# rezashkv/unlearn-ft

Hardware: AMD Instinct MI355X
Metric: bilevel train-step images/sec @512^2 pruned-SD2.1 (higher is better)
Workload: dtype bf16; 1 GPU; BASELINE configs[1] model+batch (MAC-budget-0.55 SD-2.1 student [ratio 0.556, 223.7 GMAC/img] + dense teacher [402.1 GMAC/img], B=8/GPU, 64x64 latents = 512^2 px, losses 1.0 ddpm(min-SNR 5) + 2.0 distill + 0.1 block) under the bilevel cadence of configs[2] (upper concept-suppression step every 10th iteration, second AdamW); global_batch=8, parallelism=dp1, student_params=483766084, weights=random-init, attention_precision=activation dtype, dist_backend=none, rccl_ranks=0, dp_mode=allreduce, teacher_prefetch=True

## Files before the change

include/pdmk.h:

```cpp
#ifndef PDMK_H
#define PDMK_H
#include <stdint.h>
#ifdef __cplusplus
extern "C" {
#endif

#define PDMK_F32 0
#define PDMK_BF16 1

typedef void* pdmk_stream;

int pdmk_version(void);

#define PDMK_A_ROWK 0
#define PDMK_A_CONV 1
#define PDMK_A_COLK 2
#define PDMK_B_ROWK 0
#define PDMK_B_COLK 1
#define PDMK_B_COLK_CONV 2

typedef struct pdmk_gemm_args {
    const void* A;
    const void* B;
    void* C;
// ... 24 lines not shown
    void* ln_out;
    int32_t ld_ln_out;
    float ln_eps;
} pdmk_gemm_args;
int pdmk_gemm_ln_supported(const pdmk_gemm_args* args);

#define PDMK_EPI_NONE 0
#define PDMK_EPI_GEGLU 1
#define PDMK_EPI_GEGLU_BWD 2

int pdmk_gemm(const pdmk_gemm_args* args, pdmk_stream stream);
int pdmk_conv_up2_supported(int B, int H, int W, int Ci, int Co, int dtype);
int pdmk_groupnorm_apply_colstat(const void* x, void* y, const float* gamma, const float* beta, float* stats, const int64_t* colstat,
                                 int cs_ld, int cs_col0, int B, int HW, int C, int ldx, int ldy, int G, int gs, float eps,
                                 int silu, int dtype, pdmk_stream stream);
int pdmk_up2_pack_weights(const float* w3, void* wp, void* wpt, int Co, int Ci, int dtype, pdmk_stream stream);
int pdmk_up2_combine_wgrad(const float* dwp, float* dw3, int Co, int Ci, pdmk_stream stream);
#define PDMK_COLSTAT_SCALE 1073741824.0
#define PDMK_GEMM_GROUP_MAX 8
int pdmk_gemm_group(const pdmk_gemm_args* args, int n, pdmk_stream stream, int32_t* grouped_out);
int pdmk_gemm_plan(const pdmk_gemm_args* args, pdmk_stream stream, int32_t* splitk_out);
int pdmk_gemm_last_candidate(void);
int pdmk_gemm_candidate_name(int a_mode, int b_mode, int id, char* buf, int n);
int pdmk_splitk_finish(const float* ws, void* C, const float* bias, const float* rowvec, const void* R, int64_t M,
                       int N, int ldc, int ldr, int rows_per_b, int ldrv , int nslab ,
                       int accumulate, int dtype, pdmk_stream stream);
int pdmk_splitk_finish_colstat(const float* ws, void* C, const float* bias, const float* rowvec, const void* R, int64_t M,
                               int N, int ldc, int ldr, int rows_per_b, int ldrv, int nslab, int accumulate, int64_t* colstat,
                               int cs_ld, int cs_col0, int dtype, pdmk_stream stream);
#define PDMK_SLAB_GROUP_MAX 32
typedef struct pdmk_slab_item {
    const float* ws;
    float* dst;
    int64_t n;
    int32_t nslab, pad_;
} pdmk_slab_item;
int pdmk_splitk_finish_group(const pdmk_slab_item* items, int n_items, pdmk_stream stream);
int64_t pdmk_gemm_splitk_workspace_bytes(int64_t M, int N, int splitk);

int pdmk_plan_export(const char* path);
int pdmk_plan_import(const char* path);
int pdmk_plan_size(void);
int pdmk_plan_clear(void);
int pdmk_debug_scratch_violations(void);

int pdmk_groupnorm_fwd(const void* x, void* y, const float* gamma, const float* beta, float* stats, double* ws,
// ... 159 lines not shown
```

unlearn-ft_amd/csrc/gemm.hip:

```cpp
#include <cstdio>
#include <cstdlib>
#include <cstring>
#include <map>
#include <mutex>
#include <vector>

#include "common.h"
#include <algorithm>

namespace {

#define PDMK_GEMM_NBUF 2
#ifndef PDMK_GEMM_PF2
#define PDMK_GEMM_PF2 0
#endif
constexpr int BM = 128, BN = 128;
template <typename T, int KCHUNKS, int NW> struct TileCfg {
    static constexpr int NTHREADS = 64 * NW;
    static constexpr int IM = 8 / NW * 2;
    static constexpr int TPR = NTHREADS / 128;
    static constexpr int NLD = KCHUNKS / TPR;
    static constexpr int ROW_BYTES = KCHUNKS == 8 ? 144 : 96;
    static constexpr int OPERAND_BYTES = 128 * ROW_BYTES;
    static constexpr int CH = Mma<T>::CH;
// ... 406 lines not shown
        }
    } else if (g.a_mode == PDMK_A_COLK && g.b_mode == PDMK_B_COLK) PDMK_GO(PDMK_A_COLK, PDMK_B_COLK, 0);
    else if (g.a_mode == PDMK_A_COLK && g.b_mode == PDMK_B_COLK_CONV) {
        switch (g.conv_mode) {
            case 0: PDMK_GO(PDMK_A_COLK, PDMK_B_COLK_CONV, 0); break;
            case 1: PDMK_GO(PDMK_A_COLK, PDMK_B_COLK_CONV, 1); break;
            case 2: PDMK_GO(PDMK_A_COLK, PDMK_B_COLK_CONV, 2); break;
            default: return -2;
        }
    } else return -2;
#undef PDMK_GO
    PDMK_CHECK_LAUNCH();
    return 0;
}

}

int pdmk_gemm_dma_launch(const pdmk_gemm_args& g, hipStream_t st, long a_bytes, long b_bytes);
int pdmk_gemm_ring_launch(const pdmk_gemm_args& g, hipStream_t st, long a_bytes, long b_bytes, int id);
int pdmk_gemm_ring_num_configs();
int pdmk_gemm_ring_pick(const pdmk_gemm_args& g);
int pdmk_wgrad_ring_launch(const pdmk_gemm_args& g, hipStream_t st, long a_bytes, long b_bytes, int id);
int pdmk_wgrad_ring_num_configs();

static int env_int(const char* name, int def, int* cache) {
    static int dynamic = -1;
    if (dynamic < 0) dynamic = getenv("PDMK_ENV_DYNAMIC") ? 1 : 0;
    if (*cache == INT32_MIN || dynamic) {
        const char* e = getenv(name);
        *cache = e ? atoi(e) : def;
    }
    return *cache;
}
static int dma_mode() { static int c = INT32_MIN; return env_int("PDMK_GEMM_DMA", 1, &c); }
static int ring_mode() { static int c = INT32_MIN; return env_int("PDMK_GEMM_RING", 1, &c); }
static int tune_mode() { static int c = INT32_MIN; return env_int("PDMK_GEMM_TUNE", 1, &c); }
static int forced_cfg() { static int c = INT32_MIN; return env_int("PDMK_RING_CFG", -1, &c); }
static int forced_wcfg() { static int c = INT32_MIN; return env_int("PDMK_WGRAD_CFG", -1, &c); }

namespace {

struct PlanKey {
    int v[10];
    bool operator<(const PlanKey& o) const { return memcmp(v, o.v, sizeof v) < 0; }
};
std::mutex g_plan_mu;
// ... 443 lines not shown
        char* base = reinterpret_cast<char*>(g_scratch) + off[i];
        t[i].C = base;
        t[i].ldc = a[i].N;
        t[i].colstat = nullptr;
        if (t[i].epilogue == PDMK_EPI_GEGLU_BWD) t[i].ldc = 2 * a[i].N;
        else t[i].C2 = nullptr;
        if (t[i].accumulate == 1) t[i].accumulate = 0;
        if (t[i].epilogue == PDMK_EPI_GEGLU) t[i].ldc = a[i].N / 2;
        if (t[i].colsum_out)
            t[i].colsum_out = reinterpret_cast<float*>(base + (off[i + 1] - off[i]) - (((size_t)a[i].M * 4 + 15) & ~(size_t)15));
    }
    hipEvent_t e0, e1;
    if (hipEventCreate(&e0) != hipSuccess || hipEventCreate(&e1) != hipSuccess) { (void)hipGetLastError(); return -1; }
    const float t_sep = time_us([&]() -> int {
        for (int i = 0; i < n; ++i) {
            int rc = launch_candidate(t[i], st, ids[i]);
            if (rc == 1) rc = launch_legacy(t[i], st);
            if (rc) return rc;
        }
        return 0;
    }, st, e0, e1);
    int best = -1;
    float bt = t_sep * 0.98f;
    int cands[PDMK_GEMM_GROUP_MAX + 12], nc = 0;
    for (int i = 0; i < n; ++i) cands[nc++] = ids[i];
    cands[nc++] = heuristic_cfg(a[0]);
    if (a[0].a_mode == PDMK_A_CONV)
        for (int h = 0; h < 4; ++h) cands[nc++] = 1 + 12 + h;
    if (a[0].a_mode == PDMK_A_COLK && a[0].b_mode == PDMK_B_COLK)
        for (int w = 0; w < 5; ++w) cands[nc++] = 1 + w;
    for (int i = 0; i < nc; ++i) {
        bool seen = cands[i] <= 0;
        for (int j = 0; j < i; ++j) seen = seen || cands[j] == cands[i];
        if (seen) continue;
        const float tg = time_us([&]() -> int { return group_launch(t, n, st, cands[i]); }, st, e0, e1);
        if (tg < bt) { bt = tg; best = cands[i]; }
    }
    (void)hipEventDestroy(e0);
    (void)hipEventDestroy(e1);
    if (getenv("PDMK_TUNE_LOG")) {
        fprintf(stderr, "[pdmk group] n=%d", n);
        for (int i = 0; i < n; ++i) fprintf(stderr, " (%d,%d,%d|a%d sk%d id%d)", a[i].M, a[i].N, a[i].K, a[i].a_mode, a[i].splitk, ids[i]);
        fprintf(stderr, " separate %.1f us -> %s %d (%.1f us)\n", t_sep, best > 0 ? "grouped cand" : "separate", best, best > 0 ? bt : t_sep);
    }
    {
        std::lock_guard<std::mutex> lk(g_plan_mu);
        if (!scratch_check()) return -1;
    }
    return best;
}

}

// ... 46 lines not shown
        if (can_tune(st)) {
            id = tune_group(a, n, ids, st);
            std::lock_guard<std::mutex> lk(g_plan_mu);
            g_group_plan[key] = id;
        } else {
            id = ids[0];
            for (int i = 1; i < n; ++i)
                if (ids[i] != ids[0]) id = -1;
        }
    }
    if (id > 0) {
        const int rc = group_launch(a, n, st, id);
        if (rc == 0) {
            g_last_candidate = id;
            if (grouped_out) *grouped_out = n;
            return 0;
        }
        if (rc != 1) return rc;
    }
    return separate();
}

extern "C" int pdmk_gemm_last_candidate(void) { return g_last_candidate; }
int pdmk_gemm_ring_name(int id, int conv, char* buf, int n);
int pdmk_wgrad_ring_name(int id, int conv, char* buf, int n);
extern "C" int pdmk_gemm_candidate_name(int a_mode, int b_mode, int id, char* buf, int n) {
    if (!buf || n <= 0) return -1;
    if (id <= 0) {
        snprintf(buf, n, "igemm_kernel / pdmk_dma::igemm_dma_kernel (K-step-32)");
        return 0;
    }
    if (a_mode == PDMK_A_COLK) return pdmk_wgrad_ring_name(id - 1, b_mode == PDMK_B_COLK_CONV, buf, n);
    return pdmk_gemm_ring_name(id - 1, a_mode == PDMK_A_CONV, buf, n);
}

extern "C" int pdmk_gemm_plan(const pdmk_gemm_args* a, pdmk_stream stream, int32_t* splitk_out) {
    if (!a || !splitk_out) return -1;
    const pdmk_gemm_args& g = *a;
    hipStream_t st = reinterpret_cast<hipStream_t>(stream);
    *splitk_out = 1;
    if (g.M <= 0 || g.N <= 0 || g.K <= 0) return -1;
    if ((g.N & 3) || g.epilogue) return 0;
    const bool wg = wgrad_eligible(g);
    if (g.a_mode == PDMK_A_COLK && !wg) {
        *splitk_out = heuristic_wgrad_sk(g);
        return 0;
// ... 69 lines not shown
        if (kind == 'c') g_plan_cfg[k] = val;
        else if (kind == 's') g_plan_sk[k] = val;
        ++n;
    }
    fclose(f);
    return n;
}
extern "C" int pdmk_plan_clear(void) {
    std::lock_guard<std::mutex> lk(g_plan_mu);
    g_plan_cfg.clear();
    g_plan_sk.clear();
    g_group_plan.clear();
    if (g_scratch) (void)hipFree(g_scratch);
    g_scratch = nullptr;
    g_scratch_bytes = 0;
    return 0;
}

extern "C" int pdmk_debug_scratch_violations(void) {
    std::lock_guard<std::mutex> lk(g_plan_mu);
    return g_scratch_violations;
}

extern "C" int pdmk_version(void) { return 121; }
```

unlearn-ft_amd/csrc/gemm_ring.hip:

```cpp
#include "common.h"

#include <stdio.h>
#include <stdlib.h>

#ifndef PDMK_WGRAD_XCD
#define PDMK_WGRAD_XCD 1
#endif
#ifndef PDMK_HALO_PAIRS
#define PDMK_HALO_PAIRS 1
#endif
#ifndef PDMK_RING_SPLIT_ISSUE
#define PDMK_RING_SPLIT_ISSUE 0
#endif
#ifndef PDMK_HALO_SPLIT_ISSUE
#define PDMK_HALO_SPLIT_ISSUE 1
#endif

#ifndef PDMK_PRIO
#define PDMK_PRIO 0
#endif

namespace pdmk_ring {

constexpr int BK = 64, NT = 512;
constexpr unsigned OOB = 0x80000000u;
typedef __attribute__((address_space(3))) void lds_void;
// ... 916 lines not shown
        for (int i = 0; i < IM; ++i) {
            const int m = m0 + wm * (16 * IM) + i * 16 + (lane & 15);
            if (m < g.M) unsafeAtomicAdd(g.colsum_out + m, acs[i][0]);
        }
    }
    ring_epilogue<BM, NJ, STAGES * SLOT>(g, wgc, acc, smem, m0, n0);
}

template <bool CONV, int BM, int NJ, int STAGES, int OCC>
__global__ __launch_bounds__(NT, OCC) void wgrad_ring_kernel(pdmk_gemm_args g, int lg_wo, int lg_howo, unsigned a_bytes,
                                                             unsigned b_bytes) {
    __shared__ __attribute__((aligned(1024))) unsigned char smem[wgrad_smem_bytes(BM, NJ, STAGES)];
    wgrad_ring_body<CONV, BM, NJ, STAGES, OCC>(g, lg_wo, lg_howo, a_bytes, b_bytes, PDMK_WGRAD_XCD ? lc_split_xcd() : lc_plain(), smem);
}
template <bool CONV, int BM, int NJ, int STAGES, int OCC>
__global__ __launch_bounds__(NT, OCC) void wgrad_ring_group_kernel(pdmk_gemm_group_dev gg) {
    __shared__ __attribute__((aligned(1024))) unsigned char smem[wgrad_smem_bytes(BM, NJ, STAGES)];
    int pi;
    LC wgc;
    if (!lc_group(gg, pi, wgc)) return;
    wgrad_ring_body<CONV, BM, NJ, STAGES, OCC>(gg.p[pi], gg.aux0[pi], gg.aux1[pi], gg.a_bytes[pi], gg.b_bytes[pi], wgc, smem);
}

struct Config {
    int bm, nj, stages, occ;
};
static const Config kConfigs[] = {
    {256, 4, 3, 2}, {256, 5, 3, 2}, {128, 4, 4, 2}, {128, 5, 4, 2}, {64, 4, 6, 2}, {64, 5, 5, 2},
    {128, 4, 2, 4}, {64, 4, 3, 4},  {64, 5, 2, 4},  {128, 6, 3, 2}, {64, 6, 4, 2},  {128, 5, 2, 4},
    {64, 2, 4, 4},  {128, 2, 3, 4}, {64, 3, 4, 4},
};
constexpr int kNumConfigs = sizeof(kConfigs) / sizeof(kConfigs[0]);
constexpr int kNumBase = 12;

static int halo_tile_w(const pdmk_gemm_args& g, int h, int splitk) {
    const bool phase = g.conv_mode >= 5 && g.conv_mode <= 13;
    if (g.a_mode != PDMK_A_CONV || !(g.conv_mode == 0 || phase) || g.conv_ho != g.conv_hi || g.conv_wo != g.conv_wi) return 0;
    if (phase && (h < 2 || !PDMK_HALO_PAIRS || g.R || (splitk > 1))) return 0;
    if ((g.conv_ci % 8) || g.conv_wi < 4) return 0;
    if (phase ? ((g.ldb % 8) || g.ldb < (g.conv_mode == 13 ? 16 : 4) * g.conv_ci) : g.ldb != 9 * g.conv_ci) return 0;
    if ((splitk > 1 ? splitk : 1) > (g.conv_ci + 63) / 64) return 0;
    const int bm = h < 2 ? 256 : 128, pmax = h < 2 ? 400 : 264;
    const int H = g.conv_hi, W = g.conv_wi, HW = H * W;
    if (HW < bm) return (bm % HW) == 0 && (bm / HW) * (H + 2) * (W + 2) <= pmax ? W : 0;
    if (HW % bm) return 0;
    static const int pref = getenv("PDMK_HALO_TW") ? atoi(getenv("PDMK_HALO_TW")) : 0;
// ... 417 lines not shown
        }
        return hipGetLastError() == hipSuccess ? 0 : -1000;
    }
    const Config c = kConfigs[id < kNumBase ? id : id - kNumHalo];
#define PDMK_RING_GGO(BMv, NJv, STv, OCv)                                                                             \
    case (BMv * 1000 + NJv * 100 + STv * 10 + OCv):                                                                   \
        if (conv) hipLaunchKernelGGL((igemm_ring_group_kernel<true, BMv, NJv, STv, OCv>), grid, dim3(NT), 0, st, G.gg); \
        else hipLaunchKernelGGL((igemm_ring_group_kernel<false, BMv, NJv, STv, OCv>), grid, dim3(NT), 0, st, G.gg);   \
        break;
    switch (c.bm * 1000 + c.nj * 100 + c.stages * 10 + c.occ) {
        PDMK_RING_GGO(256, 4, 3, 2) PDMK_RING_GGO(256, 5, 3, 2) PDMK_RING_GGO(128, 4, 4, 2) PDMK_RING_GGO(128, 5, 4, 2)
        PDMK_RING_GGO(64, 4, 6, 2) PDMK_RING_GGO(64, 5, 5, 2) PDMK_RING_GGO(128, 4, 2, 4) PDMK_RING_GGO(64, 4, 3, 4)
        PDMK_RING_GGO(64, 5, 2, 4) PDMK_RING_GGO(128, 6, 3, 2) PDMK_RING_GGO(64, 6, 4, 2) PDMK_RING_GGO(128, 5, 2, 4)
        PDMK_RING_GGO(64, 2, 4, 4) PDMK_RING_GGO(128, 2, 3, 4) PDMK_RING_GGO(64, 3, 4, 4)
        default: return 1;
    }
#undef PDMK_RING_GGO
    return hipGetLastError() == hipSuccess ? 0 : -1000;
}

struct WCfg { int bm, nj, stages, occ; };
static const WCfg kWCfgs[] = {{128, 4, 4, 2}, {128, 4, 2, 4}, {64, 4, 3, 4}, {128, 2, 3, 4}, {64, 2, 4, 4}};
constexpr int kNumW = sizeof(kWCfgs) / sizeof(kWCfgs[0]);
int pdmk_wgrad_ring_num_configs() { return kNumW + 2; }
int pdmk_wgrad_ring_name(int id, int conv, char* buf, int n) {
    if (id == kNumW || id == kNumW + 1) {
        snprintf(buf, n, "pdmk_ring::conv_wgrad_halo_kernel<%d, %d>", id == kNumW ? 2 : 4, id == kNumW ? 3 : 2);
        return 0;
    }
    if (id < 0 || id >= kNumW) return -1;
    const WCfg c = kWCfgs[id];
    snprintf(buf, n, "pdmk_ring::wgrad_ring_kernel<%s, %d, %d, %d, %d>", conv ? "true" : "false", c.bm, c.nj, c.stages, c.occ);
    return 0;
}
int pdmk_wgrad_ring_launch(const pdmk_gemm_args& g, hipStream_t st, long a_bytes, long b_bytes, int id) {
    using namespace pdmk_ring;
    if (g.dtype != PDMK_BF16 || g.a_mode != PDMK_A_COLK || g.b_mode == PDMK_B_ROWK || !g.out_f32) return 1;
    const bool conv = g.b_mode == PDMK_B_COLK_CONV;
    if ((g.M % 8) || (g.N % 8) || (g.lda % 8) || (!conv && (g.ldb % 8))) return 1;
    if (conv && ((g.conv_ci % 8) || (g.conv_ld % 8) || g.conv_mode == 3 || g.conv_mode == 4 || g.conv_mode > 8)) return 1;
    if (id == kNumW || id == kNumW + 1) {
        if (!wgrad_halo_ok(g)) return 1;
        const int nblk = (g.K + 127) / 128, sk = g.splitk > 1 ? g.splitk : 1, bm = id == kNumW ? 64 : 128;
        if (sk > nblk) return 1;
        dim3 grid(((g.M + bm - 1) / bm) * ((g.conv_ci + 63) / 64), sk);
        if (bm == 64) hipLaunchKernelGGL((conv_wgrad_halo_kernel<2, 3>), grid, dim3(NT), 0, st, g, (unsigned)a_bytes, (unsigned)b_bytes);
        else hipLaunchKernelGGL((conv_wgrad_halo_kernel<4, 2>), grid, dim3(NT), 0, st, g, (unsigned)a_bytes, (unsigned)b_bytes);
        return hipGetLastError() == hipSuccess ? 0 : -1000;
    }
    if (id < 0 || id >= kNumW) return 1;
    int lg_wo = -1, lg_howo = -1;
    if (conv) {
        auto lg = [](int v) { int l = 0; if (v <= 0 || (v & (v - 1))) return -1; while ((1 << l) < v) ++l; return l; };
        lg_wo = lg(g.conv_wo);
        lg_howo = lg(g.conv_ho * g.conv_wo);
        if (lg_wo < 0 || lg_howo < 0) lg_wo = lg_howo = -1;
    }
    const WCfg c = kWCfgs[id];
    const int bn = 32 * c.nj;
    dim3 grid(((g.M + c.bm - 1) / c.bm) * ((g.N + bn - 1) / bn), g.splitk > 1 ? g.splitk : 1);
#define PDMK_WG_GO(BMv, NJv, STv, OCv)                                                                                \
    case (BMv * 1000 + NJv * 100 + STv * 10 + OCv):                                                                   \
        if (conv) hipLaunchKernelGGL((wgrad_ring_kernel<true, BMv, NJv, STv, OCv>), grid, dim3(NT), 0, st, g, lg_wo,  \
                                     lg_howo, (unsigned)a_bytes, (unsigned)b_bytes);                                  \
        else hipLaunchKernelGGL((wgrad_ring_kernel<false, BMv, NJv, STv, OCv>), grid, dim3(NT), 0, st, g, lg_wo,      \
                                lg_howo, (unsigned)a_bytes, (unsigned)b_bytes);                                       \
        break;
    switch (c.bm * 1000 + c.nj * 100 + c.stages * 10 + c.occ) {
        PDMK_WG_GO(128, 4, 4, 2) PDMK_WG_GO(128, 4, 2, 4) PDMK_WG_GO(64, 4, 3, 4) PDMK_WG_GO(128, 2, 3, 4) PDMK_WG_GO(64, 2, 4, 4)
        default: return 1;
    }
#undef PDMK_WG_GO
    return hipGetLastError() == hipSuccess ? 0 : -1000;
}

int pdmk_wgrad_ring_group_launch(const pdmk_gemm_args* gs, int n, hipStream_t st, const long* a_bytes, const long* b_bytes, int id) {
    using namespace pdmk_ring;
    if (n < 2 || n > PDMK_GEMM_GROUP_MAX || id < 0 || id > kNumW + 1) return 1;
    const bool conv = gs[0].b_mode == PDMK_B_COLK_CONV;
    const bool halo = id == kNumW || id == kNumW + 1;
    GroupGrid G;
    for (int i = 0; i < n; ++i) {
        const pdmk_gemm_args& g = gs[i];
        if (g.dtype != PDMK_BF16 || g.a_mode != PDMK_A_COLK || g.b_mode == PDMK_B_ROWK || !g.out_f32) return 1;
        if ((g.b_mode == PDMK_B_COLK_CONV) != conv) return 1;
        if ((g.M % 8) || (g.N % 8) || (g.lda % 8) || (!conv && (g.ldb % 8))) return 1;
        if (conv && ((g.conv_ci % 8) || (g.conv_ld % 8) || g.conv_mode == 3 || g.conv_mode == 4 || g.conv_mode > 8)) return 1;
        const int sk = g.splitk > 1 ? g.splitk : 1;
        if (halo) {
            if (!wgrad_halo_ok(g)) return 1;
            const int nblk = (g.K + 127) / 128, bm = id == kNumW ? 64 : 128;
            if (sk > nblk) return 1;
            G.add(i, g, ((g.M + bm - 1) / bm) * ((g.conv_ci + 63) / 64), sk, a_bytes[i], b_bytes[i]);
        } else {
            int lg_wo = -1, lg_howo = -1;
            if (conv) {
                auto lg = [](int v) { int l = 0; if (v <= 0 || (v & (v - 1))) return -1; while ((1 << l) < v) ++l; return l; };
                lg_wo = lg(g.conv_wo);
                lg_howo = lg(g.conv_ho * g.conv_wo);
                if (lg_wo < 0 || lg_howo < 0) lg_wo = lg_howo = -1;
            }
            const WCfg c = kWCfgs[id];
            const int bn = 32 * c.nj;
            G.add(i, g, ((g.M + c.bm - 1) / c.bm) * ((g.N + bn - 1) / bn), sk, a_bytes[i], b_bytes[i], lg_wo, lg_howo);
        }
    }
    G.finish(n);
    const dim3 grid(G.total);
    if (halo) {
        if (id == kNumW) hipLaunchKernelGGL((conv_wgrad_halo_group_kernel<2, 3>), grid, dim3(NT), 0, st, G.gg);
        else hipLaunchKernelGGL((conv_wgrad_halo_group_kernel<4, 2>), grid, dim3(NT), 0, st, G.gg);
        return hipGetLastError() == hipSuccess ? 0 : -1000;
    }
    const WCfg c = kWCfgs[id];
#define PDMK_WG_GGO(BMv, NJv, STv, OCv)                                                                               \
    case (BMv * 1000 + NJv * 100 + STv * 10 + OCv):                                                                   \
        if (conv) hipLaunchKernelGGL((wgrad_ring_group_kernel<true, BMv, NJv, STv, OCv>), grid, dim3(NT), 0, st, G.gg); \
        else hipLaunchKernelGGL((wgrad_ring_group_kernel<false, BMv, NJv, STv, OCv>), grid, dim3(NT), 0, st, G.gg);   \
        break;
    switch (c.bm * 1000 + c.nj * 100 + c.stages * 10 + c.occ) {
        PDMK_WG_GGO(128, 4, 4, 2) PDMK_WG_GGO(128, 4, 2, 4) PDMK_WG_GGO(64, 4, 3, 4) PDMK_WG_GGO(128, 2, 3, 4) PDMK_WG_GGO(64, 2, 4, 4)
        default: return 1;
    }
#undef PDMK_WG_GGO
    return hipGetLastError() == hipSuccess ? 0 : -1000;
}
```

unlearn-ft_amd/pdm/_pdmk.py:

```python
import ctypes as C
import os

import torch

_HERE = os.path.dirname(os.path.abspath(__file__))
LIB_PATH = os.environ.get("PDMK_LIB") or os.path.join(os.path.dirname(_HERE), "libpdmk.so")

F32, BF16 = 0, 1
EPI_NONE, EPI_GEGLU, EPI_GEGLU_BWD = 0, 1, 2
A_ROWK, A_CONV, A_COLK = 0, 1, 2
B_ROWK, B_COLK, B_COLK_CONV = 0, 1, 2


class PdmkError(RuntimeError):
    pass


def _load():
    if not os.path.exists(LIB_PATH):
        raise PdmkError(f"libpdmk.so not found at {LIB_PATH}: build it with `python __graft_entry__.py` "
                        f"(or `make -C unlearn-ft_amd/csrc`); there is no CPU/PyTorch fallback for the hot path")
    return C.CDLL(LIB_PATH)


# ... 10 lines not shown
                ("conv_b", i32), ("conv_hi", i32), ("conv_wi", i32), ("conv_ci", i32), ("conv_ho", i32),
                ("conv_wo", i32), ("conv_mode", i32), ("conv_ld", i32),
                ("dtype", i32), ("out_f32", i32), ("accumulate", i32), ("splitk", i32), ("alpha", f32), ("ldrv", i32),
                ("epilogue", i32), ("ldc2", i32), ("C2", vp), ("colstat", vp), ("cs_ld", i32), ("cs_col0", i32),
                ("ln_gamma", vp), ("ln_beta", vp), ("ln_stats", vp), ("ln_out", vp), ("ld_ln_out", i32), ("ln_eps", f32)]


class PlmsRow(C.Structure):
    _fields_ = [("t", i64), ("mode", i32), ("nterms", i32), ("wslot", i32), ("rslot", i32 * 3), ("coef", f32 * 4),
                ("v_x", f32), ("v_v", f32), ("eps_scale", f32), ("x_scale", f32), ("vpred", i32), ("pad_", i32)]


_SIGS = {
    "pdmk_version": ([], i32),
    "pdmk_gemm": ([C.POINTER(GemmArgs), vp], i32),
    "pdmk_gemm_group": ([C.POINTER(GemmArgs), i32, vp, C.POINTER(i32)], i32),
    "pdmk_gemm_plan": ([C.POINTER(GemmArgs), vp, C.POINTER(i32)], i32),
    "pdmk_gemm_ln_supported": ([C.POINTER(GemmArgs)], i32),
    "pdmk_conv_up2_supported": ([i32, i32, i32, i32, i32, i32], i32),
    "pdmk_up2_pack_weights": ([vp, vp, vp, i32, i32, i32, vp], i32),
    "pdmk_up2_combine_wgrad": ([vp, vp, i32, i32, vp], i32),
    "pdmk_gemm_last_candidate": ([], i32),
    "pdmk_gemm_candidate_name": ([i32, i32, i32, C.c_char_p, i32], i32),
    "pdmk_splitk_finish": ([vp, vp, vp, vp, vp, i64, i32, i32, i32, i32, i32, i32, i32, i32, vp], i32),
    "pdmk_splitk_finish_colstat": ([vp, vp, vp, vp, vp, i64, i32, i32, i32, i32, i32, i32, i32, vp, i32, i32, i32, vp], i32),
    "pdmk_groupnorm_fwd": ([vp, vp, vp, vp, vp, vp, i32, i32, i32, i32, i32, i32, i32, f32, i32, i32, vp], i32),
    "pdmk_groupnorm_apply_colstat": ([vp, vp, vp, vp, vp, vp, i32, i32, i32, i32, i32, i32, i32, i32, i32, f32, i32, i32, vp], i32),
    "pdmk_groupnorm_bwd": ([vp, vp, vp, vp, vp, vp, vp, vp, vp, vp, i64, i32, i32, i32, i32, i32, i32, i32, i32, i32, i32, vp, i32, i32, vp], i32),
    "pdmk_groupnorm_bwd_partial_dims": ([i32, i32, i32, i32, i32, i32, C.POINTER(i32), C.POINTER(i32)], i32),
    "pdmk_layernorm_bwd_partial_dims": ([i32, i32, C.POINTER(i32), C.POINTER(i32)], i32),
    "pdmk_reduce_partials_group": ([vp, i32, vp], i32),
    "pdmk_splitk_finish_group": ([vp, i32, vp], i32),
    "pdmk_layernorm_fwd": ([vp, vp, vp, vp, vp, i32, i32, i32, i32, f32, i32, vp], i32),
    "pdmk_layernorm_bwd": ([vp, vp, vp, vp, vp, vp, vp, vp, i64, i32, i32, i32, i32, i32, i32, vp, i32, i32, vp], i32),
    "pdmk_attn_fwd": ([vp, vp, vp, vp, vp, i32, i32, i32, i32, i64, i32, i64, i32, i64, i32, i64, i32, f32, i32, vp], i32),
    "pdmk_attn_bwd": ([vp, vp, vp, vp, vp, vp, vp, vp, vp, vp, i32, i32, i32, i32,
                       i64, i32, i64, i32, i64, i32, i64, i32, i64, i32, i64, i32, i64, i32, f32, vp, i64, i32, vp], i32),
    "pdmk_geglu_fwd": ([vp, vp, i32, i32, i32, i32, i32, i32, vp], i32),
    "pdmk_geglu_bwd": ([vp, vp, vp, i32, i32, i32, i32, i32, i32, i32, vp], i32),
    "pdmk_quantize_e4m3": ([vp, vp, i64, i32, vp], i32),
    "pdmk_silu_fwd": ([vp, vp, i64, i32, vp], i32),
    "pdmk_silu_bwd": ([vp, vp, vp, i64, i32, vp], i32),
    "pdmk_copy2d": ([vp, vp, i64, i32, i32, i32, i32, i32, vp], i32),
    "pdmk_cast_permute": ([vp, vp, i32, i32, i32, i32, i32, vp], i32),
    "pdmk_colsum": ([vp, vp, i64, i32, i32, i32, i32, i32, i32, vp], i32),
    "pdmk_pool2x2_sum": ([vp, vp, i32, i32, i32, i32, i32, vp], i32),
# ... 349 lines not shown


def zero_(t):
    assert t.is_contiguous() and (t.numel() * t.element_size()) % 16 == 0
    _chk(_lib.pdmk_zero(_p(t), t.numel() * t.element_size(), _st()), "pdmk_zero")
    return t


def attn_last_forms():
    w = int(_lib.pdmk_attn_last_forms())
    return w & 15, (w >> 4) & 15, (w >> 8) & 15, w >> 12


def last_candidate():
    return int(_lib.pdmk_gemm_last_candidate())


def candidate_name(a_mode, b_mode, cand):
    buf = C.create_string_buffer(160)
    _chk(_lib.pdmk_gemm_candidate_name(a_mode, b_mode, cand, buf, 160), "pdmk_gemm_candidate_name")
    return buf.value.decode()


def splitk_plan(A, B, M, N, K, lda, ldb, a_mode=A_ROWK, conv=None):
    g = GemmArgs()
    g.A, g.B = _p(A), _p(B)
    g.M, g.N, g.K = M, N, K
    g.lda, g.ldb, g.ldc = lda, ldb, N
    g.a_mode, g.b_mode = a_mode, B_ROWK
    if conv is not None:
        (g.conv_b, g.conv_hi, g.conv_wi, g.conv_ci, g.conv_ho, g.conv_wo, g.conv_mode, g.conv_ld) = conv
    g.dtype = dt(A)
    g.splitk, g.alpha = 1, 1.0
    sk = i32(1)
    _chk(_lib.pdmk_gemm_plan(C.byref(g), _st(), C.byref(sk)), "pdmk_gemm_plan")
    return int(sk.value)


def wgrad_plan(dy, x, M, N, K, lda, ldb, b_mode=B_COLK, conv=None, slabs=False):
    g = GemmArgs()
    g.accumulate = 2 if slabs else 0
    g.A, g.B = _p(dy), _p(x)
    g.M, g.N, g.K = M, N, K
    g.lda, g.ldb, g.ldc = lda, ldb, N
    g.a_mode, g.b_mode = A_COLK, b_mode
    if conv is not None:
# ... 59 lines not shown
            _chk(_lib.pdmk_splitk_finish_group(C.cast(arr, vp), len(chunk), _st()), "pdmk_splitk_finish_group")
        self.bytes = 0


def wgrad(dy, x, dW, M, N, K, lda, ldb, *, b_mode=B_COLK, conv=None, colsum_out=None, macs=None, queue=None):
    if queue is not None and (M * N) % 4 == 0 and dW.is_contiguous():
        sk = wgrad_plan(dy, x, M, N, K, lda, ldb, b_mode, conv, slabs=True)
        if sk > 1:
            if queue.full():
                queue.flush()
            ws = torch.empty(sk * M * N, device=dy.device, dtype=torch.float32)
            gemm(dy, x, ws, M, N, K, lda, ldb, N, a_mode=A_COLK, b_mode=b_mode, conv=conv, out_f32=True, splitk=sk,
                 accumulate=2, dtype=dt(x), macs=macs, colsum_out=colsum_out)
            queue.add(ws, dW, M * N, sk)
            return
    else:
        sk = wgrad_plan(dy, x, M, N, K, lda, ldb, b_mode, conv)
    gemm(dy, x, dW, M, N, K, lda, ldb, N, a_mode=A_COLK, b_mode=b_mode, conv=conv, out_f32=True, splitk=sk,
         accumulate=(sk == 1), dtype=dt(x), macs=macs, colsum_out=colsum_out)


_WG_TARGET = int(os.environ.get("PDMK_WG_TARGET", "512"))
_WG_MINK = int(os.environ.get("PDMK_WG_MINK", "32"))
_WG_CONV_SLABS = os.environ.get("PDMK_WGRAD_SLABS_CONV", "0") == "1"


def wgrad_group(items, queue, target_wgs=None):
    items = [tuple(it) + (B_COLK, None) if len(it) == 10 else tuple(it) for it in items]
    while items:
        K, bm = items[0][5], items[0][10]
        same = [it for it in items if it[5] == K and it[10] == bm][:GROUP_MAX]
        items = [it for it in items if not any(it is s_ for s_ in same)]
        conv_g = bm == B_COLK_CONV
        tiles = sum(((it[3] + 127) // 128) * ((it[4] + 127) // 128) for it in same)
        nk = max(1, K // 64)
        sk = max(1, min((target_wgs or _WG_TARGET) // max(tiles, 1), nk // _WG_MINK, 64))
        if len(same) == 1 or (queue is None and not conv_g):
            for dy, x, dW, M, N, K_, lda, ldb, cs, macs, bm_, conv in same:
                wgrad(dy, x, dW, M, N, K_, lda, ldb, b_mode=bm_, conv=conv, colsum_out=cs, macs=macs, queue=None if conv_g else queue)
            continue
        with Recorder() as r:
            slabs = []
            for dy, x, dW, M, N, K_, lda, ldb, cs, macs, bm_, conv in same:
                if (not conv_g or _WG_CONV_SLABS) and queue is not None and sk > 1 and (M * N) % 4 == 0 and dW.is_contiguous():
                    ws = torch.empty(sk * M * N, device=dy.device, dtype=torch.float32)
                    gemm(dy, x, ws, M, N, K_, lda, ldb, N, a_mode=A_COLK, b_mode=bm_, conv=conv, out_f32=True, splitk=sk, accumulate=2,
                         dtype=dt(x), macs=macs, colsum_out=cs)
                    slabs.append((ws, dW, M * N, sk))
                else:
                    ska = sk if conv_g else 1
                    gemm(dy, x, dW, M, N, K_, lda, ldb, N, a_mode=A_COLK, b_mode=bm_, conv=conv, out_f32=True, splitk=ska,
                         accumulate=(ska == 1), dtype=dt(x), macs=macs, colsum_out=cs)
        gemm_group(r.recs)
        for ws, dW, n, nslab in slabs:
            if queue.full():
                queue.flush()
            queue.add(ws, dW, n, nslab)


@_recordable("groupnorm_apply_colstat")
def groupnorm_apply_colstat(x, y, gamma, beta, stats, colstat, col0, B, HW, Cc, ldx, ldy, G, gs, eps, silu):
    _chk(_lib.pdmk_groupnorm_apply_colstat(_p(x), _p(y), _p(gamma), _p(beta), _p(stats), _p(colstat), colstat.shape[2], int(col0),
                                           B, HW, Cc, ldx, ldy, G, gs, eps, int(silu), dt(x), _st()),
# ... 450 lines not shown
```

Before: 190.6 images/s.

## Add wide-tile wgrad GEMM kernels and autotune split-K for grouped weight gradients

Adds a new wgrad GEMM kernel family with larger output tiles (256x128, 320x128, 128x256, 128x320, 256x256) and multi-stage LDS rings. These kernels are registered as extra grouped-launch candidates for the autotuner. The Python grouped-wgrad path now times several split-K choices, derived from the tile counts of the candidate tile shapes, charges each a cost for the slab reduction, and caches the fastest per shape key. The goal is more operand reuse per workgroup and a better balance between split-K parallelism and reduction overhead. The cost is more compiled kernels, more tuning time on first use, and higher register and LDS pressure.

```diff
diff --git a/include/pdmk.h b/include/pdmk.h
--- a/include/pdmk.h
+++ b/include/pdmk.h
@@ -70,6 +70,8 @@
 int pdmk_gemm_plan(const pdmk_gemm_args* args, pdmk_stream stream, int32_t* splitk_out);
 int pdmk_gemm_last_candidate(void);
 int pdmk_gemm_candidate_name(int a_mode, int b_mode, int id, char* buf, int n);
+int pdmk_wgrad_num_candidates(void);
+int pdmk_wgrad_candidate_tile(int cand, int32_t* bm, int32_t* bn);
 int pdmk_splitk_finish(const float* ws, void* C, const float* bias, const float* rowvec, const void* R, int64_t M,
                        int N, int ldc, int ldr, int rows_per_b, int ldrv , int nslab ,
                        int accumulate, int dtype, pdmk_stream stream);
diff --git a/unlearn-ft_amd/csrc/gemm.hip b/unlearn-ft_amd/csrc/gemm.hip
--- a/unlearn-ft_amd/csrc/gemm.hip
+++ b/unlearn-ft_amd/csrc/gemm.hip
@@ -452,6 +452,7 @@
 int pdmk_gemm_ring_pick(const pdmk_gemm_args& g);
 int pdmk_wgrad_ring_launch(const pdmk_gemm_args& g, hipStream_t st, long a_bytes, long b_bytes, int id);
 int pdmk_wgrad_ring_num_configs();
+int pdmk_wgrad_ring_tile(int id, int* bm, int* bn);
 
 static int env_int(const char* name, int def, int* cache) {
     static int dynamic = -1;
@@ -941,13 +942,14 @@
     }, st, e0, e1);
     int best = -1;
     float bt = t_sep * 0.98f;
-    int cands[PDMK_GEMM_GROUP_MAX + 12], nc = 0;
+    int cands[PDMK_GEMM_GROUP_MAX + 24], nc = 0;
     for (int i = 0; i < n; ++i) cands[nc++] = ids[i];
     cands[nc++] = heuristic_cfg(a[0]);
     if (a[0].a_mode == PDMK_A_CONV)
         for (int h = 0; h < 4; ++h) cands[nc++] = 1 + 12 + h;
     if (a[0].a_mode == PDMK_A_COLK && a[0].b_mode == PDMK_B_COLK)
-        for (int w = 0; w < 5; ++w) cands[nc++] = 1 + w;
+        for (int w = 0; w < pdmk_wgrad_ring_num_configs(); ++w)
+            if (w < 5 || w >= 7) cands[nc++] = 1 + w;
     for (int i = 0; i < nc; ++i) {
         bool seen = cands[i] <= 0;
         for (int j = 0; j < i; ++j) seen = seen || cands[j] == cands[i];
@@ -1040,6 +1042,15 @@
 }
 
 extern "C" int pdmk_gemm_last_candidate(void) { return g_last_candidate; }
+extern "C" int pdmk_wgrad_candidate_tile(int cand, int32_t* bm, int32_t* bn) {
+    if (!bm || !bn || cand < 1) return -1;
+    int m = 0, n = 0;
+    if (pdmk_wgrad_ring_tile(cand - 1, &m, &n)) return -1;
+    *bm = m;
+    *bn = n;
+    return 0;
+}
+extern "C" int pdmk_wgrad_num_candidates(void) { return 1 + pdmk_wgrad_ring_num_configs(); }
 int pdmk_gemm_ring_name(int id, int conv, char* buf, int n);
 int pdmk_wgrad_ring_name(int id, int conv, char* buf, int n);
 extern "C" int pdmk_gemm_candidate_name(int a_mode, int b_mode, int id, char* buf, int n) {
@@ -1155,4 +1166,4 @@
     return g_scratch_violations;
 }
 
-extern "C" int pdmk_version(void) { return 121; }
+extern "C" int pdmk_version(void) { return 122; }
diff --git a/unlearn-ft_amd/csrc/gemm_ring.hip b/unlearn-ft_amd/csrc/gemm_ring.hip
--- a/unlearn-ft_amd/csrc/gemm_ring.hip
+++ b/unlearn-ft_amd/csrc/gemm_ring.hip
@@ -2,6 +2,8 @@
 
 #include <stdio.h>
 #include <stdlib.h>
+
+#include <utility>
 
 #ifndef PDMK_WGRAD_XCD
 #define PDMK_WGRAD_XCD 1
@@ -964,6 +966,238 @@
     wgrad_ring_body<CONV, BM, NJ, STAGES, OCC>(gg.p[pi], gg.aux0[pi], gg.aux1[pi], gg.a_bytes[pi], gg.b_bytes[pi], wgc, smem);
 }
 
+constexpr int wide_units(int T) { return (T + 127) / 128; }
+constexpr int wide_unit_w(int T, int u) { return T - 128 * u >= 128 ? 128 : 64; }
+constexpr int wgrad_wide_smem_bytes(int BMT, int BNT, int STAGES) { return STAGES * 128 * (BMT + BNT); }
+
+template <int BMT, int BNT, int LDS_BYTES, int UAi, int UBi>
+__device__ __forceinline__ void wgrad_wide_epilogue_pair(const pdmk_gemm_args& g, const LC wgc,
+                                                         f32x4 (&acc)[wide_units(BMT)][wide_units(BNT)][2][4], unsigned char* smem,
+                                                         int m0, int n0) {
+    constexpr int WA = wide_unit_w(BMT, UAi), WB = wide_unit_w(BNT, UBi);
+    const int m0u = m0 + 128 * UAi, n0u = n0 + 128 * UBi;
+    if (m0u >= g.M || n0u >= g.N) return;
+    f32x4 t[WA / 64][WB / 32];
+#pragma unroll
+    for (int i = 0; i < WA / 64; ++i)
+#pragma unroll
+        for (int j = 0; j < WB / 32; ++j) t[i][j] = acc[UAi][UBi][i][j];
+    ring_epilogue<WA, WB / 32, LDS_BYTES>(g, wgc, t, smem, m0u, n0u);
+}
+template <int BMT, int BNT, int LDS_BYTES, int... P>
+__device__ __forceinline__ void wgrad_wide_epilogue(const pdmk_gemm_args& g, const LC wgc,
+                                                    f32x4 (&acc)[wide_units(BMT)][wide_units(BNT)][2][4], unsigned char* smem, int m0,
+                                                    int n0, std::integer_sequence<int, P...>) {
+    (wgrad_wide_epilogue_pair<BMT, BNT, LDS_BYTES, P / wide_units(BNT), P % wide_units(BNT)>(g, wgc, acc, smem, m0, n0), ...);
+}
+
+template <bool CONV, int BMT, int BNT, int STAGES>
+__device__ __forceinline__ void wgrad_wide_body(const pdmk_gemm_args& g, int lg_wo, int lg_howo, unsigned a_bytes, unsigned b_bytes,
+                                                const LC wgc, unsigned char* smem) {
+    typedef Mma<bf16> MM;
+    constexpr int UA = wide_units(BMT), UB = wide_units(BNT);
+    constexpr int A_BYTES = 128 * BMT, B_BYTES = 128 * BNT, SLOT = A_BYTES + B_BYTES;
+    constexpr int PT = SLOT / 1024 / 8;
+    static_assert(BMT % 64 == 0 && BNT % 64 == 0 && BMT >= 128 && BNT >= 128, "tile");
+    static_assert(STAGES >= 2 && STAGES * SLOT <= 160 * 1024, "the ring must fit the 160 KiB LDS");
+    static_assert(STAGES * SLOT == wgrad_wide_smem_bytes(BMT, BNT, STAGES), "smem size of the kernel wrappers");
+    static_assert((STAGES - 2) * PT <= 63, "s_waitcnt vmcnt immediate");
+
+    const int tid = threadIdx.x, lane = tid & 63, wave = __builtin_amdgcn_readfirstlane(tid >> 6);
+    const int wm = wave >> 1, wn = wave & 1;
+    const int ntn = (g.N + BNT - 1) / BNT;
+    const int tile = xcd_remap(wgc.bx, wgc.gx);
+    const int m0 = (tile / ntn) * BMT, n0 = (tile % ntn) * BNT;
+    const int nk_total = (g.K + BK - 1) / BK;
+    const int per = (nk_total + wgc.gy - 1) / wgc.gy;
+    const int kt0 = wgc.by * per;
+    const int kt1 = min(nk_total, kt0 + per);
+    if (kt0 >= kt1 && g.accumulate != 2) return;
+
+    const auto rsrcA = __builtin_amdgcn_make_buffer_rsrc(const_cast<void*>(g.A), (short)0, (int)a_bytes, 0x00020000);
+    const auto rsrcB = __builtin_amdgcn_make_buffer_rsrc(const_cast<void*>(g.B), (short)0, (int)b_bytes, 0x00020000);
+    const ConvGeom cg{g.conv_hi, g.conv_wi, g.conv_ci, g.conv_ho, g.conv_wo, g.conv_ld, g.conv_mode};
+
+    auto lane_row = [&](int rbytes) { return rbytes == 256 ? (lane >> 4) : (lane >> 3); };
+    auto lane_lc = [&](int rbytes) {
+        if (rbytes == 256) return (lane & 15) ^ (((lane >> 4) | (((wave >> 1) & 1) << 2)) << 1);
+        return (lane & 7) ^ (((((lane >> 3) >> 1) & 1) | ((wave & 1) << 1)) << 1);
+    };
+    int acol[UA], bcol[UB], b_tap[UB], b_ci[UB];
+#pragma unroll
+    for (int u = 0; u < UA; ++u) acol[u] = m0 + 128 * u + lane_lc(2 * wide_unit_w(BMT, u)) * 8;
+#pragma unroll
+    for (int u = 0; u < UB; ++u) {
+        bcol[u] = n0 + 128 * u + lane_lc(2 * wide_unit_w(BNT, u)) * 8;
+        b_tap[u] = b_ci[u] = 0;
+        if (CONV) {
+            b_tap[u] = bcol[u] / cg.ci;
+            b_ci[u] = bcol[u] - b_tap[u] * cg.ci;
+        }
+    }
+
+    auto issue = [&](int kt, int slot) {
+        unsigned char* sa = smem + slot * SLOT;
+#pragma unroll
+        for (int u = 0; u < UA; ++u) {
+            const int R = 2 * wide_unit_w(BMT, u);
+            const bool a_ok = acol[u] < g.M;
+#pragma unroll
+            for (int i = 0; i < 2; ++i) {
+                if (i * 8 * 1024 >= 64 * R) continue;
+                const int piece = i * 8 + wave;
+                const int kr = kt * BK + piece * (1024 / R) + lane_row(R);
+                unsigned krs = (unsigned)kr;
+                if (CONV && cg.mode >= 5 && kr < g.K) {
+                    const int hw = cg.ho * cg.wo, b = kr / hw, rem = kr - b * hw, oy = rem / cg.wo, ox = rem - oy * cg.wo;
+                    const int ph = cg.mode - 5;
+                    krs = (unsigned)((b * 2 * cg.ho + 2 * oy + (ph >> 1)) * (2 * cg.wo) + 2 * ox + (ph & 1));
+                }
+                const unsigned va = (kr < g.K && a_ok) ? (krs * (unsigned)g.lda + (unsigned)acol[u]) * 2u : OOB;
+                __builtin_amdgcn_raw_ptr_buffer_load_lds(rsrcA, (lds_void*)(sa + 16384 * u + piece * 1024), 16, (int)va, 0, 0, 0);
+            }
+        }
+#pragma unroll
+        for (int u = 0; u < UB; ++u) {
+            const int R = 2 * wide_unit_w(BNT, u);
+            const bool b_ok = bcol[u] < g.N;
+#pragma unroll
+            for (int i = 0; i < 2; ++i) {
+                if (i * 8 * 1024 >= 64 * R) continue;
+                const int piece = i * 8 + wave;
+                const int kr = kt * BK + piece * (1024 / R) + lane_row(R);
+                const bool kok = kr < g.K;
+                unsigned vb = OOB;
+                if (CONV) {
+                    if (kok && b_ok) {
+                        int b, oy, ox;
+                        if (lg_wo >= 0) {
+                            b = kr >> lg_howo;
+                            const int rem = kr & ((1 << lg_howo) - 1);
+                            oy = rem >> lg_wo;
+                            ox = rem & ((1 << lg_wo) - 1);
+                        } else {
+                            const int hw = cg.ho * cg.wo;
+                            b = kr / hw;
+                            const int rem = kr - b * hw;
+                            oy = rem / cg.wo;
+                            ox = rem - oy * cg.wo;
+                        }
+                        const int px = conv_src_pixel(cg, b, oy, ox, b_tap[u]);
+                        if (px >= 0) vb = ((unsigned)px * (unsigned)cg.ld + (unsigned)b_ci[u]) * 2u;
+                    }
+                } else if (kok && b_ok) {
+                    vb = ((unsigned)kr * (unsigned)g.ldb + (unsigned)bcol[u]) * 2u;
+                }
+                __builtin_amdgcn_raw_ptr_buffer_load_lds(rsrcB, (lds_void*)(sa + A_BYTES + 16384 * u + piece * 1024), 16, (int)vb, 0, 0, 0);
+            }
+        }
+    };
+
+    f32x4 acc[UA][UB][2][4], acs[UA][2];
+#pragma unroll
+    for (int ua = 0; ua < UA; ++ua)
+#pragma unroll
+        for (int i = 0; i < 2; ++i) {
+            acs[ua][i] = f32x4{0.f, 0.f, 0.f, 0.f};
+#pragma unroll
+            for (int ub = 0; ub < UB; ++ub)
+#pragma unroll
+                for (int j = 0; j < 4; ++j) acc[ua][ub][i][j] = f32x4{0.f, 0.f, 0.f, 0.f};
+        }
+    const bool do_colsum = g.colsum_out != nullptr && n0 == 0 && wn == 0;
+    bf16x8 ones;
+#pragma unroll
+    for (int e = 0; e < 8; ++e) ones[e] = (bf16)1.0f;
+
+    const int tg = lane >> 4, tq = (lane & 15) >> 2, tp = lane & 3;
+    const int f256 = (tq | ((tg & 1) << 2)) << 1, f128 = (((tq >> 1) & 1) | ((tg & 1) << 1)) << 1;
+    typedef __attribute__((address_space(3))) s16x4 lds_s16x4;
+    auto tr_frag = [&](const unsigned char* base, int rbytes, int kk, int col0) -> bf16x8 {
+        const unsigned ch = (unsigned)(((col0 >> 3) ^ (rbytes == 256 ? f256 : f128)) | (tp >> 1));
+        const unsigned char* a0 = base + (unsigned)(kk + 8 * tg + tq) * (unsigned)rbytes + ch * 16u + (unsigned)(tp & 1) * 8u;
+        s16x4 lo = __builtin_amdgcn_ds_read_tr16_b64_v4i16((lds_s16x4*)(a0));
+        s16x4 hi = __builtin_amdgcn_ds_read_tr16_b64_v4i16((lds_s16x4*)(a0 + 4 * rbytes));
+        s16x8 v = __builtin_shufflevector(lo, hi, 0, 1, 2, 3, 4, 5, 6, 7);
+        return __builtin_bit_cast(bf16x8, v);
+    };
+
+#pragma unroll
+    for (int s = 0; s < STAGES - 1; ++s)
+        if (kt0 + s < kt1) issue(kt0 + s, s);
+
+    int slot = 0;
+    for (int kt = kt0; kt < kt1; ++kt) {
+        if (STAGES == 2) asm volatile("s_waitcnt vmcnt(0)" ::: "memory");
+        else if (kt + STAGES - 1 <= kt1) asm volatile("s_waitcnt vmcnt(%0)" ::"n"((STAGES - 2) * PT) : "memory");
+        else wait_vmcnt_dyn(min(STAGES - 2, kt1 - 1 - kt) * PT);
+        __builtin_amdgcn_s_barrier();
+        if (kt + STAGES - 1 < kt1) issue(kt + STAGES - 1, slot == 0 ? STAGES - 1 : slot - 1);
+        const unsigned char* sa = smem + slot * SLOT;
+        const unsigned char* sb = sa + A_BYTES;
+#pragma unroll
+        for (int kk = 0; kk < BK; kk += 32) {
+            bf16x8 af[UA][2];
+#pragma unroll
+            for (int ua = 0; ua < UA; ++ua) {
+                const int W = wide_unit_w(BMT, ua), IMu = W / 64;
+#pragma unroll
+                for (int i = 0; i < 2; ++i)
+                    if (i < IMu) af[ua][i] = tr_frag(sa + 16384 * ua, 2 * W, kk, wm * (16 * IMu) + i * 16);
+            }
+#pragma unroll
+            for (int ub = 0; ub < UB; ++ub) {
+                const int W = wide_unit_w(BNT, ub), NJu = W / 32;
+                bf16x8 bf[4];
+#pragma unroll
+                for (int j = 0; j < 4; ++j)
+                    if (j < NJu) bf[j] = tr_frag(sb + 16384 * ub, 2 * W, kk, wn * (16 * NJu) + j * 16);
+#pragma unroll
+                for (int ua = 0; ua < UA; ++ua)
+#pragma unroll
+                    for (int i = 0; i < 2; ++i)
+#pragma unroll
+                        for (int j = 0; j < 4; ++j)
+                            if (i < wide_unit_w(BMT, ua) / 64 && j < NJu) acc[ua][ub][i][j] = MM::mma(bf[j], af[ua][i], acc[ua][ub][i][j]);
+            }
+            if (do_colsum) {
+#pragma unroll
+                for (int ua = 0; ua < UA; ++ua)
+#pragma unroll
+                    for (int i = 0; i < 2; ++i)
+                        if (i < wide_unit_w(BMT, ua) / 64) acs[ua][i] = MM::mma(ones, af[ua][i], acs[ua][i]);
+            }
+        }
+        slot = slot + 1 == STAGES ? 0 : slot + 1;
+    }
+    if (do_colsum && (lane >> 4) == 0) {
+#pragma unroll
+        for (int ua = 0; ua < UA; ++ua) {
+            const int IMu = wide_unit_w(BMT, ua) / 64;
+#pragma unroll
+            for (int i = 0; i < 2; ++i) {
+                const int m = m0 + 128 * ua + wm * (16 * IMu) + i * 16 + (lane & 15);
+                if (i < IMu && m < g.M) unsafeAtomicAdd(g.colsum_out + m, acs[ua][i][0]);
+            }
+        }
+    }
+    wgrad_wide_epilogue<BMT, BNT, STAGES * SLOT>(g, wgc, acc, smem, m0, n0, std::make_integer_sequence<int, UA * UB>{});
+}
+
+template <bool CONV, int BMT, int BNT, int STAGES>
+__global__ __launch_bounds__(NT, 2) void wgrad_wide_kernel(pdmk_gemm_args g, int lg_wo, int lg_howo, unsigned a_bytes, unsigned b_bytes) {
+    __shared__ __attribute__((aligned(1024))) unsigned char smem[wgrad_wide_smem_bytes(BMT, BNT, STAGES)];
+    wgrad_wide_body<CONV, BMT, BNT, STAGES>(g, lg_wo, lg_howo, a_bytes, b_bytes, PDMK_WGRAD_XCD ? lc_split_xcd() : lc_plain(), smem);
+}
+template <bool CONV, int BMT, int BNT, int STAGES>
+__global__ __launch_bounds__(NT, 2) void wgrad_wide_group_kernel(pdmk_gemm_group_dev gg) {
+    __shared__ __attribute__((aligned(1024))) unsigned char smem[wgrad_wide_smem_bytes(BMT, BNT, STAGES)];
+    int pi;
+    LC wgc;
+    if (!lc_group(gg, pi, wgc)) return;
+    wgrad_wide_body<CONV, BMT, BNT, STAGES>(gg.p[pi], gg.aux0[pi], gg.aux1[pi], gg.a_bytes[pi], gg.b_bytes[pi], wgc, smem);
+}
+
 struct Config {
     int bm, nj, stages, occ;
 };
@@ -1427,8 +1661,24 @@
 struct WCfg { int bm, nj, stages, occ; };
 static const WCfg kWCfgs[] = {{128, 4, 4, 2}, {128, 4, 2, 4}, {64, 4, 3, 4}, {128, 2, 3, 4}, {64, 2, 4, 4}};
 constexpr int kNumW = sizeof(kWCfgs) / sizeof(kWCfgs[0]);
-int pdmk_wgrad_ring_num_configs() { return kNumW + 2; }
+struct WWide { int bm, bn, stages; };
+static const WWide kWWide[] = {{256, 128, 3}, {320, 128, 2}, {128, 256, 3}, {128, 320, 2}, {256, 256, 2}};
+constexpr int kNumWide = sizeof(kWWide) / sizeof(kWWide[0]);
+constexpr int kWideBase = kNumW + 2;
+int pdmk_wgrad_ring_num_configs() { return kNumW + 2 + kNumWide; }
+int pdmk_wgrad_ring_tile(int id, int* bm, int* bn) {
+    if (id < 0 || id >= kWideBase + kNumWide) return -1;
+    if (id < kNumW) { *bm = kWCfgs[id].bm; *bn = 32 * kWCfgs[id].nj; }
+    else if (id < kWideBase) { *bm = id == kNumW ? 64 : 128; *bn = 9 * 64; }
+    else { *bm = kWWide[id - kWideBase].bm; *bn = kWWide[id - kWideBase].bn; }
+    return 0;
+}
 int pdmk_wgrad_ring_name(int id, int conv, char* buf, int n) {
+    if (id >= kWideBase && id < kWideBase + kNumWide) {
+        const WWide c = kWWide[id - kWideBase];
+        snprintf(buf, n, "pdmk_ring::wgrad_wide_kernel<%s, %d, %d, %d>", conv ? "true" : "false", c.bm, c.bn, c.stages);
+        return 0;
+    }
     if (id == kNumW || id == kNumW + 1) {
         snprintf(buf, n, "pdmk_ring::conv_wgrad_halo_kernel<%d, %d>", id == kNumW ? 2 : 4, id == kNumW ? 3 : 2);
         return 0;
@@ -1453,13 +1703,30 @@
         else hipLaunchKernelGGL((conv_wgrad_halo_kernel<4, 2>), grid, dim3(NT), 0, st, g, (unsigned)a_bytes, (unsigned)b_bytes);
         return hipGetLastError() == hipSuccess ? 0 : -1000;
     }
-    if (id < 0 || id >= kNumW) return 1;
+    if (id < 0 || id >= kWideBase + kNumWide) return 1;
     int lg_wo = -1, lg_howo = -1;
     if (conv) {
         auto lg = [](int v) { int l = 0; if (v <= 0 || (v & (v - 1))) return -1; while ((1 << l) < v) ++l; return l; };
         lg_wo = lg(g.conv_wo);
         lg_howo = lg(g.conv_ho * g.conv_wo);
         if (lg_wo < 0 || lg_howo < 0) lg_wo = lg_howo = -1;
+    }
+    if (id >= kWideBase) {
+        const WWide c = kWWide[id - kWideBase];
+        dim3 grid(((g.M + c.bm - 1) / c.bm) * ((g.N + c.bn - 1) / c.bn), g.splitk > 1 ? g.splitk : 1);
+#define PDMK_WW_GO(BMv, BNv, STv)                                                                                     \
+    case (BMv * 10000 + BNv * 10 + STv):                                                                              \
+        if (conv) hipLaunchKernelGGL((wgrad_wide_kernel<true, BMv, BNv, STv>), grid, dim3(NT), 0, st, g, lg_wo,       \
+                                     lg_howo, (unsigned)a_bytes, (unsigned)b_bytes);                                  \
+        else hipLaunchKernelGGL((wgrad_wide_kernel<false, BMv, BNv, STv>), grid, dim3(NT), 0, st, g, lg_wo,           \
+                                lg_howo, (unsigned)a_bytes, (unsigned)b_bytes);                                       \
+        break;
+        switch (c.bm * 10000 + c.bn * 10 + c.stages) {
+            PDMK_WW_GO(256, 128, 3) PDMK_WW_GO(320, 128, 2) PDMK_WW_GO(128, 256, 3) PDMK_WW_GO(128, 320, 2) PDMK_WW_GO(256, 256, 2)
+            default: return 1;
+        }
+#undef PDMK_WW_GO
+        return hipGetLastError() == hipSuccess ? 0 : -1000;
     }
     const WCfg c = kWCfgs[id];
     const int bn = 32 * c.nj;
@@ -1481,9 +1748,10 @@
 
 int pdmk_wgrad_ring_group_launch(const pdmk_gemm_args* gs, int n, hipStream_t st, const long* a_bytes, const long* b_bytes, int id) {
     using namespace pdmk_ring;
-    if (n < 2 || n > PDMK_GEMM_GROUP_MAX || id < 0 || id > kNumW + 1) return 1;
+    if (n < 2 || n > PDMK_GEMM_GROUP_MAX || id < 0 || id >= kWideBase + kNumWide) return 1;
     const bool conv = gs[0].b_mode == PDMK_B_COLK_CONV;
     const bool halo = id == kNumW || id == kNumW + 1;
+    const bool wide = id >= kWideBase;
     GroupGrid G;
     for (int i = 0; i < n; ++i) {
         const pdmk_gemm_args& g = gs[i];
@@ -1505,9 +1773,9 @@
                 lg_howo = lg(g.conv_ho * g.conv_wo);
                 if (lg_wo < 0 || lg_howo < 0) lg_wo = lg_howo = -1;
             }
-            const WCfg c = kWCfgs[id];
-            const int bn = 32 * c.nj;
-            G.add(i, g, ((g.M + c.bm - 1) / c.bm) * ((g.N + bn - 1) / bn), sk, a_bytes[i], b_bytes[i], lg_wo, lg_howo);
+            int bm, bn;
+            pdmk_wgrad_ring_tile(id, &bm, &bn);
+            G.add(i, g, ((g.M + bm - 1) / bm) * ((g.N + bn - 1) / bn), sk, a_bytes[i], b_bytes[i], lg_wo, lg_howo);
         }
     }
     G.finish(n);
@@ -1515,6 +1783,20 @@
     if (halo) {
         if (id == kNumW) hipLaunchKernelGGL((conv_wgrad_halo_group_kernel<2, 3>), grid, dim3(NT), 0, st, G.gg);
         else hipLaunchKernelGGL((conv_wgrad_halo_group_kernel<4, 2>), grid, dim3(NT), 0, st, G.gg);
+        return hipGetLastError() == hipSuccess ? 0 : -1000;
+    }
+    if (wide) {
+        const WWide c = kWWide[id - kWideBase];
+#define PDMK_WW_GGO(BMv, BNv, STv)                                                                                    \
+    case (BMv * 10000 + BNv * 10 + STv):                                                                              \
+        if (conv) hipLaunchKernelGGL((wgrad_wide_group_kernel<true, BMv, BNv, STv>), grid, dim3(NT), 0, st, G.gg);    \
+        else hipLaunchKernelGGL((wgrad_wide_group_kernel<false, BMv, BNv, STv>), grid, dim3(NT), 0, st, G.gg);        \
+        break;
+        switch (c.bm * 10000 + c.bn * 10 + c.stages) {
+            PDMK_WW_GGO(256, 128, 3) PDMK_WW_GGO(320, 128, 2) PDMK_WW_GGO(128, 256, 3) PDMK_WW_GGO(128, 320, 2) PDMK_WW_GGO(256, 256, 2)
+            default: return 1;
+        }
+#undef PDMK_WW_GGO
         return hipGetLastError() == hipSuccess ? 0 : -1000;
     }
     const WCfg c = kWCfgs[id];
diff --git a/unlearn-ft_amd/pdm/_pdmk.py b/unlearn-ft_amd/pdm/_pdmk.py
--- a/unlearn-ft_amd/pdm/_pdmk.py
+++ b/unlearn-ft_amd/pdm/_pdmk.py
@@ -1,5 +1,6 @@
 import ctypes as C
 import os
+import sys
 
 import torch
 
@@ -56,6 +57,8 @@
     "pdmk_up2_combine_wgrad": ([vp, vp, i32, i32, vp], i32),
     "pdmk_gemm_last_candidate": ([], i32),
     "pdmk_gemm_candidate_name": ([i32, i32, i32, C.c_char_p, i32], i32),
+    "pdmk_wgrad_num_candidates": ([], i32),
+    "pdmk_wgrad_candidate_tile": ([i32, C.POINTER(i32), C.POINTER(i32)], i32),
     "pdmk_splitk_finish": ([vp, vp, vp, vp, vp, i64, i32, i32, i32, i32, i32, i32, i32, i32, vp], i32),
     "pdmk_splitk_finish_colstat": ([vp, vp, vp, vp, vp, i64, i32, i32, i32, i32, i32, i32, i32, vp, i32, i32, i32, vp], i32),
     "pdmk_groupnorm_fwd": ([vp, vp, vp, vp, vp, vp, i32, i32, i32, i32, i32, i32, i32, f32, i32, i32, vp], i32),
@@ -451,6 +454,15 @@
     return buf.value.decode()
 
 
+def wgrad_candidate_tiles():
+    out = {}
+    for cand in range(1, int(_lib.pdmk_wgrad_num_candidates())):
+        bm, bn = i32(0), i32(0)
+        _chk(_lib.pdmk_wgrad_candidate_tile(cand, C.byref(bm), C.byref(bn)), "pdmk_wgrad_candidate_tile")
+        out[cand] = (int(bm.value), int(bn.value))
+    return out
+
+
 def splitk_plan(A, B, M, N, K, lda, ldb, a_mode=A_ROWK, conv=None):
     g = GemmArgs()
     g.A, g.B = _p(A), _p(B)
@@ -556,7 +568,47 @@
 
 _WG_TARGET = int(os.environ.get("PDMK_WG_TARGET", "512"))
 _WG_MINK = int(os.environ.get("PDMK_WG_MINK", "32"))
+_WG_SPLIT_TUNE = os.environ.get("PDMK_WG_SPLIT_TUNE", "1") != "0"
 _WG_CONV_SLABS = os.environ.get("PDMK_WGRAD_SLABS_CONV", "0") == "1"
+
+
+_WG_SPLIT = {}
+
+
+def wgrad_group_splits(shapes, K, target, linear=True):
+    nk = max(1, K // 64)
+    out = []
+    tiles_of = [(128, 128)] + [t for c, t in sorted(wgrad_candidate_tiles().items()) if linear and t[1] != 9 * 64 and t[0] * t[1] > 128 * 128]
+    for bm, bn in tiles_of:
+        tiles = sum(((M + bm - 1) // bm) * ((N + bn - 1) // bn) for M, N in shapes)
+        sk = max(1, min(target // max(tiles, 1), nk // _WG_MINK, 64))
+        if sk not in out:
+            out.append(sk)
+    return out
+
+
+def _wg_group_time(same, sk, reps=3):
+    with Recorder() as r:
+        for dy, x, dW, M, N, K_, lda, ldb, cs, macs, bm_, conv in same:
+            ws = torch.empty(sk * M * N, device=dy.device, dtype=torch.float32)
+            gemm(dy, x, ws, M, N, K_, lda, ldb, N, a_mode=A_COLK, b_mode=bm_, conv=conv, out_f32=True, splitk=sk,
+                 accumulate=2 if sk > 1 else 0, dtype=dt(x), macs=macs)
+    prof = globals()["PROFILE"]
+    globals()["PROFILE"] = None
+    try:
+        gemm_group(r.recs)
+        best = float("inf")
+        for _ in range(2):
+            e0, e1 = torch.cuda.Event(enable_timing=True), torch.cuda.Event(enable_timing=True)
+            e0.record()
+            for _ in range(reps):
+                gemm_group(r.recs)
+            e1.record()
+            e1.synchronize()
+            best = min(best, e0.elapsed_time(e1) * 1000.0 / reps)
+    finally:
+        globals()["PROFILE"] = prof
+    return best + (sum((sk + 1) * it[3] * it[4] * 4.0 for it in same) / 4.0e6 if sk > 1 else 0.0)
 
 
 def wgrad_group(items, queue, target_wgs=None):
@@ -566,13 +618,27 @@
         same = [it for it in items if it[5] == K and it[10] == bm][:GROUP_MAX]
         items = [it for it in items if not any(it is s_ for s_ in same)]
         conv_g = bm == B_COLK_CONV
-        tiles = sum(((it[3] + 127) // 128) * ((it[4] + 127) // 128) for it in same)
-        nk = max(1, K // 64)
-        sk = max(1, min((target_wgs or _WG_TARGET) // max(tiles, 1), nk // _WG_MINK, 64))
+        target = target_wgs or _WG_TARGET
+        shapes = [(it[3], it[4]) for it in same]
+        sk = wgrad_group_splits(shapes, K, target, linear=False)[0]
         if len(same) == 1 or (queue is None and not conv_g):
             for dy, x, dW, M, N, K_, lda, ldb, cs, macs, bm_, conv in same:
                 wgrad(dy, x, dW, M, N, K_, lda, ldb, b_mode=bm_, conv=conv, colsum_out=cs, macs=macs, queue=None if conv_g else queue)
             continue
+        slab_ok = all((it[3] * it[4]) % 4 == 0 and it[2].is_contiguous() for it in same)
+        if not conv_g and slab_ok and _WG_SPLIT_TUNE:
+            key = (target, K, tuple((it[3], it[4], it[6], it[7]) for it in same))
+            if key in _WG_SPLIT:
+                sk = _WG_SPLIT[key]
+            elif RECORD is None and not torch.cuda.is_current_stream_capturing():
+                opts = wgrad_group_splits(shapes, K, target)
+                if len(opts) > 1:
+                    times = [_wg_group_time(same, o) for o in opts]
+                    sk = opts[times.index(min(times))]
+                    if os.environ.get("PDMK_TUNE_LOG"):
+                        print(f"[pdmk wgrad_group] {shapes} K={K}: splits {opts} -> {[round(t, 1) for t in times]} us -> {sk}",
+                              file=sys.stderr)
+                _WG_SPLIT[key] = sk
         with Recorder() as r:
             slabs = []
             for dy, x, dW, M, N, K_, lda, ldb, cs, macs, bm_, conv in same:
```

Measured after the change: 191.6 images/s (median of 6 runs). Within noise of the previous version (+0.5%).
